# JackWoo0831/Yolov7-tracker

Measured on NVIDIA H100. Metric: tracked_frames_per_sec, higher is better.
Workload: dtype fp16

## Files before the change

### yolov7-tracker_b200/b200track/conv.py

```python
import ctypes as C

import torch

from . import _lib as L


def pack_conv_weight(w, cin_pad=None, dtype=torch.bfloat16):
    cout, cin, kh, kw = w.shape
    cin_pad = cin_pad or (cin + 15) // 16 * 16
    rows = (cout + 15) // 16 * 16
    out = torch.zeros((rows, kh, kw, cin_pad), dtype=torch.float32, device=w.device)
    out[:cout, :, :, :cin] = w.permute(0, 2, 3, 1)
    return out.reshape(rows, kh * kw * cin_pad).to(dtype).contiguous()


def pack_conv_weight_rowpack(w, dtype=torch.bfloat16):
    cout, cin, kh, kw = w.shape
    assert kh == 3 and kw == 3 and cin <= 16
    rows = (cout + 15) // 16 * 16
    out = torch.zeros((rows, 3, 4, 16), dtype=torch.float32, device=w.device)
    out[:cout, :, :3, :cin] = w.permute(0, 2, 3, 1)
    return out.reshape(rows, 192).to(dtype).contiguous()


class ConvPlan:
    def __init__(self, x, w_packed, bias, y, n, h, w, cin, in_coff, cout, k, stride, out_coff, act=True, out_f32=False,
                 block_n=0, tile_w=0, stages=0, in_row_pixels=0, rowpack=False, x_pixel0=0, halo=False, mt=1, splits=1, halo_bufs=0, producers=0, tps=0, out_bufs=0, kpair=0):
        self.lib = L.load()
        assert x.dtype in (torch.bfloat16, torch.float16) and x.is_contiguous() and y.is_contiguous()
        assert w_packed.dtype == x.dtype and bias.dtype == torch.float32 and (out_f32 or y.dtype == x.dtype)
        self.keep = (x, w_packed, bias, y)
        self.geom = dict(n=n, h=h, w=w, cin=cin, cout=cout, k=k, stride=stride, out_f32=bool(out_f32), rowpack=bool(rowpack))
        d = L.ConvDesc(x=x.data_ptr() + x_pixel0 * x.shape[-1] * 2, w_packed=w_packed.data_ptr(), bias=bias.data_ptr(), y=y.data_ptr(), n=n, h=h, w=w,
                       cin=cin, in_pitch=x.shape[-1], in_coff=in_coff, cout=cout, cout_rows=w_packed.shape[0], kh=k, kw=k,
                       stride=stride, out_pitch=y.shape[-1], out_coff=out_coff, act=int(act), out_f32=int(out_f32),
                       block_n=block_n, tile_w=tile_w, stages=stages, in_row_pixels=in_row_pixels, rowpack=int(rowpack), io_dtype=L.act_dtype_code(x.dtype),
                       halo=int(halo), halo_bufs=int(halo_bufs), tps=int(tps), kpair=int(kpair), out_bufs=int(out_bufs), mt=int(mt), producers=int(producers), splits=int(splits))
        self.handle = C.c_void_p()
        rc = self.lib.b2t_conv_plan_create(C.byref(d), C.byref(self.handle))
        if rc != 0:
            raise L.B2TError("b2t_conv_plan_create: %s" % (self.lib.b2t_conv_last_error() or b"").decode())
        self.flops = self.lib.b2t_conv_plan_flops(self.handle)
        info = (C.c_int * 17)()
        self.lib.b2t_conv_plan_info(self.handle, info, 17)
        self.info = dict(zip(("grid", "threads", "smem", "bn", "stages", "mt", "splits", "halo", "halo_bufs", "tiles_m", "tiles_n", "acc_regs", "producers", "tps", "b_res", "out_bufs", "kpair"), list(info)))

    def run(self, stream=None):
        s = C.c_void_p(torch.cuda.current_stream().cuda_stream if stream is None else stream)
        rc = self.lib.b2t_conv_run(self.handle, s)
        if rc != 0:
            raise L.B2TError("b2t_conv_run: %s" % (self.lib.b2t_conv_last_error() or b"").decode())

    def __del__(self):
        try:
            if self.handle:
                self.lib.b2t_conv_plan_destroy(self.handle)
                self.handle = None
        except Exception:
            pass
```

### yolov7-tracker_b200/csrc/b2t_conv.cu

```cuda
#include <cuda.h>
#include <cuda_runtime.h>
#include <cuda_bf16.h>
#include <cuda_fp16.h>
#include <stdint.h>
#include <string>
#include <cstdio>
#include <cstdlib>
#include "../../include/b200track.h"
#include "b2t_wgmma.cuh"

namespace {

constexpr int kMaxStages = 8;
constexpr int kTileM = 128;
constexpr int kMaxHalo = 3;
constexpr int kRing = 4;
constexpr int kMaxProducers = 2;

struct ConvParams {
    int N, H, W, Cin;
    int Ho, Wo, Cout;
    int KH, KW, stride, pad;
    int pad_w;
    int halo;
    int halo_bytes;
    int halo_bufs;
    int kpair;
    int tps;
    int b_res;
    int out_bufs;
    int MT;
    int sub_off;
    int TH, TW;
    int BK;
    int BN;
    int tiles_w, tiles_h;
    int out_pitch;
    int out_coff;
    int act;
    float act_floor, act_slope;
    int out_f32;
    int f16;
    int flat;
    int stages;
    int tiles_m, tiles_n;
    int P;
    int splits;
    int ksteps;
    long long total_pix;
    float* ws;
    int* flags;
};

__device__ __forceinline__ uint32_t smem_u32(const void* p) { return (uint32_t)__cvta_generic_to_shared(p); }

__device__ __forceinline__ void mbar_init(uint64_t* bar, int count) {
    asm volatile("mbarrier.init.shared::cta.b64 [%0], %1;" ::"r"(smem_u32(bar)), "r"(count));
}
__device__ __forceinline__ void mbar_expect_tx(uint64_t* bar, uint32_t bytes) {
    asm volatile("mbarrier.arrive.expect_tx.shared::cta.b64 _, [%0], %1;" ::"r"(smem_u32(bar)), "r"(bytes) : "memory");
}
__device__ __forceinline__ void mbar_arrive(uint64_t* bar) {
    asm volatile("mbarrier.arrive.shared::cta.b64 _, [%0];" ::"r"(smem_u32(bar)) : "memory");
}
__device__ __forceinline__ void mbar_wait(uint64_t* bar, uint32_t parity) {
    asm volatile(
        "{\n\t.reg .pred p;\n\t"
        "WAIT_%=:\n\t"
        "mbarrier.try_wait.parity.shared::cta.b64 p, [%0], %1;\n\t"
        "@p bra DONE_%=;\n\t"
        "bra WAIT_%=;\n\t"
        "DONE_%=:\n\t}" ::"r"(smem_u32(bar)), "r"(parity) : "memory");
}
__device__ __forceinline__ void tma_load_4d(void* dst, const CUtensorMap* map, uint64_t* bar, int c0, int c1, int c2, int c3) {
    asm volatile(
        "cp.async.bulk.tensor.4d.shared::cluster.global.tile.mbarrier::complete_tx::bytes [%0], [%1, {%3, %4, %5, %6}], [%2];"
        ::"r"(smem_u32(dst)), "l"(map), "r"(smem_u32(bar)), "r"(c0), "r"(c1), "r"(c2), "r"(c3) : "memory");
}
__device__ __forceinline__ void tma_load_2d(void* dst, const CUtensorMap* map, uint64_t* bar, int c0, int c1) {
    asm volatile(
        "cp.async.bulk.tensor.2d.shared::cluster.global.tile.mbarrier::complete_tx::bytes [%0], [%1, {%3, %4}], [%2];"
        ::"r"(smem_u32(dst)), "l"(map), "r"(smem_u32(bar)), "r"(c0), "r"(c1) : "memory");
}
__device__ __forceinline__ void tma_load_3d(void* dst, const CUtensorMap* map, uint64_t* bar, int c0, int c1, int c2) {
    asm volatile(
        "cp.async.bulk.tensor.3d.shared::cluster.global.tile.mbarrier::complete_tx::bytes [%0], [%1, {%3, %4, %5}], [%2];"
        ::"r"(smem_u32(dst)), "l"(map), "r"(smem_u32(bar)), "r"(c0), "r"(c1), "r"(c2) : "memory");
}
__device__ __forceinline__ void tma_store_4d(const CUtensorMap* map, const void* src, int c0, int c1, int c2, int c3) {
    asm volatile("cp.async.bulk.tensor.4d.global.shared::cta.bulk_group [%0, {%2, %3, %4, %5}], [%1];"
                 ::"l"(map), "r"(smem_u32(src)), "r"(c0), "r"(c1), "r"(c2), "r"(c3) : "memory");
}
__device__ __forceinline__ void tma_store_2d(const CUtensorMap* map, const void* src, int c0, int c1) {
    asm volatile("cp.async.bulk.tensor.2d.global.shared::cta.bulk_group [%0, {%2, %3}], [%1];"
                 ::"l"(map), "r"(smem_u32(src)), "r"(c0), "r"(c1) : "memory");
}
__device__ __forceinline__ bool elect_one() {
    uint32_t pred;
    asm volatile("{\n\t.reg .pred p;\n\telect.sync _|p, 0xffffffff;\n\tselp.u32 %0, 1, 0, p;\n\t}" : "=r"(pred));
    return pred != 0;
}
__device__ __forceinline__ void wgmma_fence() { asm volatile("wgmma.fence.sync.aligned;" ::: "memory"); }
__device__ __forceinline__ void wgmma_commit() { asm volatile("wgmma.commit_group.sync.aligned;" ::: "memory"); }
template <int N> __device__ __forceinline__ void wgmma_wait() { asm volatile("wgmma.wait_group.sync.aligned %0;" ::"n"(N) : "memory"); }
template <int R> __device__ __forceinline__ void acc_fence(float (&d)[R]) {
#pragma unroll
    for (int i = 0; i < R; ++i) asm volatile("" : "+f"(d[i])::"memory");
}

__device__ __forceinline__ float silu(float v) {
    const float h = 0.5f * v;
    float t;
    asm("tanh.approx.f32 %0, %1;" : "=f"(t) : "f"(h));
    return fmaf(h, t, h);
}

__device__ __forceinline__ uint32_t pack16(float a, float b, bool f16) {
    if (f16) { const __half2 h = __floats2half2_rn(a, b); return *reinterpret_cast<const uint32_t*>(&h); }
    const __nv_bfloat162 h = __floats2bfloat162_rn(a, b); return *reinterpret_cast<const uint32_t*>(&h);
}

template <bool F32, bool F16, int BN>
__device__ __forceinline__ void stage_box(const float (&acc)[BN / 2], int bx, const float* __restrict__ bias_c, uint8_t* box, int r0, int lane,
                                          int act, float floor_v, float slope_v) {
    constexpr int cpb = F32 ? 32 : 64;
    const int cq = 2 * (lane & 3);
#pragma unroll
    for (int j = 0; j < BN / 8; ++j) {
        if ((8 * j) / cpb != bx) continue;
        const int col = 8 * j + cq;
        const float2 b = __ldg(reinterpret_cast<const float2*>(bias_c + col));
#pragma unroll
        for (int h = 0; h < 2; ++h) {
            const int r = r0 + 8 * h;
            float v0 = acc[4 * j + 2 * h] + b.x, v1 = acc[4 * j + 2 * h + 1] + b.y;
            if (act) { v0 = silu(v0); v1 = silu(v1); }
            else {
                v0 = fmaxf(fmaxf(v0, floor_v), v0 * slope_v); v1 = fmaxf(fmaxf(v1, floor_v), v1 * slope_v);
            }
            const int byte = (col - bx * cpb) * (F32 ? 4 : 2);
            uint8_t* dst = box + r * 128 + ((((byte >> 4) ^ (r & 7)) << 4) | (byte & 15));
            if (F32) *reinterpret_cast<float2*>(dst) = make_float2(v0, v1);
            else *reinterpret_cast<uint32_t*>(dst) = pack16(v0, v1, F16);
        }
    }
}

template <bool F32, bool F16, int MT, int BN>
__global__ void __launch_bounds__(256 * MT + 32 * kMaxProducers, (MT == 1 && BN <= 64) ? 2 : 1)
conv_bias_act_kernel(const __grid_constant__ CUtensorMap map_a, const __grid_constant__ CUtensorMap map_b,
                     const __grid_constant__ CUtensorMap map_c, const float* __restrict__ bias, int* __restrict__ sched,
                     const ConvParams p) {
    extern __shared__ __align__(1024) uint8_t smem[];
    constexpr int kConsumerWarps = 8 * MT;
    const int warp = threadIdx.x >> 5, lane = threadIdx.x & 31;
    const int a_bytes = kTileM * p.BK * 2;
    const int b_bytes = BN * p.BK * 2;
    const int stage_bytes = (((p.halo ? p.tps * b_bytes : (MT * a_bytes + b_bytes) * p.kpair) + 1023) / 1024) * 1024;
    uint8_t* tiles = smem + ((1024u - (smem_u32(smem) & 1023u)) & 1023u);
    uint8_t* ring = tiles + (p.halo ? p.halo_bufs * p.halo_bytes : 0);
    const int kStages = p.stages;
    constexpr int box_bytes = kTileM * 128;
    const int staging_bytes = p.out_bufs * box_bytes;
    uint8_t* stage_out = ring + kStages * stage_bytes;
    uint64_t* full_bar = reinterpret_cast<uint64_t*>(stage_out + MT * staging_bytes);
    uint64_t* empty_bar = full_bar + kMaxStages;
    uint64_t* ring_full = empty_bar + kMaxStages;
    uint64_t* ring_empty = ring_full + kRing;
    uint64_t* a_full = ring_empty + kRing;
    uint64_t* a_empty = a_full + kMaxHalo;
    int* tile_ring = reinterpret_cast<int*>(a_empty + kMaxHalo);
    int* last_flag = tile_ring + kRing;
    int* first_unit = last_flag + 2;

    const int ntaps = p.KH * p.KW;
    const int total_units = p.tiles_m * p.tiles_n * p.splits;
    const int P = p.P;
    const int pw = warp - kConsumerWarps;

    asm volatile("griddepcontrol.launch_dependents;" ::: "memory");
    if (pw == 0 && lane == 0) {
        *first_unit = atomicAdd(sched, 1);
        asm volatile("prefetch.tensormap [%0];" ::"l"(&map_a) : "memory");
        asm volatile("prefetch.tensormap [%0];" ::"l"(&map_b) : "memory");
        asm volatile("prefetch.tensormap [%0];" ::"l"(&map_c) : "memory");
        for (int s = 0; s < kStages; ++s) { mbar_init(&full_bar[s], 1); mbar_init(&empty_bar[s], 2 * MT); }
        for (int r = 0; r < kRing; ++r) { mbar_init(&ring_full[r], 1); mbar_init(&ring_empty[r], P - 1 + kConsumerWarps); }
        for (int h = 0; h < kMaxHalo; ++h) { mbar_init(&a_full[h], 1); mbar_init(&a_empty[h], 2 * MT); }
        asm volatile("fence.mbarrier_init.release.cluster;" ::: "memory");
    }
    __syncthreads();

    auto unit_coords = [&](int u, int& n0, int& img, int& ho0, int& wo0, long long& pix0, int& k0, int& k1) {
        int t = u;
        k0 = 0; k1 = p.ksteps;
        if (p.splits > 1) {
            t = u / p.splits;
            const int sp = u - t * p.splits;
            k0 = (p.ksteps * sp) / p.splits;
            k1 = (p.ksteps * (sp + 1)) / p.splits;
        }
        const int mt = t / p.tiles_n, nt = t % p.tiles_n;
        n0 = nt * BN; img = 0; ho0 = 0; wo0 = 0; pix0 = 0;
        if (p.flat) pix0 = (long long)mt * (kTileM * MT);
        else {
            const int per_img = p.tiles_w * p.tiles_h;
            img = mt / per_img;
            const int r = mt % per_img;
            ho0 = (r / p.tiles_w) * (p.halo ? p.TH : p.TH * MT);
            wo0 = (r % p.tiles_w) * (p.halo ? p.TW * MT : p.TW);
        }
    };

    if (pw >= 0) {
        int stage = 0; uint32_t phase = 0;
        int hbuf = 0; uint32_t hphase = 0;
        int rslot = 0; uint32_t rphase = 0;
        int c = 0;
        int u = *first_unit;
        const int groups = p.halo ? 9 / p.tps : 1;
        auto load_b = [&](int st, int n0, int k0, int s) {
            uint8_t* sb = ring + st * stage_bytes + (p.halo ? 0 : MT * a_bytes * p.kpair);
            if (p.halo) {
                const int kc = k0 + s / groups, tap = (s % groups) * p.tps;
                if (p.tps == 1) tma_load_2d(sb, &map_b, &full_bar[st], tap * p.Cin + kc * p.BK, n0);
                else tma_load_3d(sb, &map_b, &full_bar[st], kc * p.BK, n0, tap);
            } else if (p.kpair == 2) {
                tma_load_3d(sb, &map_b, &full_bar[st], 0, n0, 2 * (k0 + s));
            } else {
                const int kt = k0 + s, kc = kt / ntaps, tap = kt % ntaps;
                tma_load_2d(sb, &map_b, &full_bar[st], tap * p.Cin + kc * p.BK, n0);
            }
        };
        const uint32_t stage_tx = (uint32_t)(p.halo ? p.tps * b_bytes : (MT * a_bytes + b_bytes) * p.kpair);
        int npre = 0;
        if (u < total_units) {
            int n0, img, ho0, wo0, k0, k1; long long pix0;
            unit_coords(u, n0, img, ho0, wo0, pix0, k0, k1);
            if (p.b_res) {
                if (pw == 0 && elect_one()) {
                    mbar_expect_tx(&full_bar[0], (uint32_t)(9 * b_bytes));
                    tma_load_3d(ring, &map_b, &full_bar[0], 0, n0, 0);
                }
            } else {
                const int nsteps = (k1 - k0) * groups;
                npre = nsteps < kStages ? nsteps : kStages;
                for (int s = pw; s < npre; s += P)
                    if (elect_one()) {
                        mbar_expect_tx(&full_bar[s], stage_tx);
                        load_b(s, n0, k0, s);
                    }
            }
            __syncwarp();
        }
        asm volatile("griddepcontrol.wait;" ::: "memory");
        for (;;) {
            if (pw == 0) {
                const bool live = u < total_units;
                mbar_wait(&ring_empty[rslot], rphase ^ 1);
                if (lane == 0) {
                    tile_ring[rslot] = live ? u : -1;
                    mbar_arrive(&ring_full[rslot]);
                }
                __syncwarp();
                if (++rslot == kRing) { rslot = 0; rphase ^= 1; }
                if (!live) break;
            } else {
                mbar_wait(&ring_full[rslot], rphase);
                u = tile_ring[rslot];
                __syncwarp();
                if (lane == 0) mbar_arrive(&ring_empty[rslot]);
                if (++rslot == kRing) { rslot = 0; rphase ^= 1; }
                if (u < 0) break;
            }
            int next = 0;
            if (pw == 0) {
                if (lane == 0) next = atomicAdd(sched, 1);
                next = __shfl_sync(0xffffffffu, next, 0);
            }
            int n0, img, ho0, wo0, k0, k1; long long pix0;
            unit_coords(u, n0, img, ho0, wo0, pix0, k0, k1);
            if (p.halo) {
                const uint32_t halo_tx = (uint32_t)((p.TW * MT + 2) * (p.TH + 2) * p.BK * 2);
                auto load_halo = [&](int kc) {
                    mbar_wait(&a_empty[hbuf], hphase ^ 1);
                    if (elect_one()) {
                        mbar_expect_tx(&a_full[hbuf], halo_tx);
                        tma_load_4d(tiles + hbuf * p.halo_bytes, &map_a, &a_full[hbuf], kc * p.BK, wo0 - 1, ho0 - 1, img);
                    }
                    __syncwarp();
                    if (++hbuf == p.halo_bufs) { hbuf = 0; hphase ^= 1; }
                };
                if (pw == 0) load_halo(k0);
                for (int kc = k0; kc < k1; ++kc) {
                    if (pw == 0 && kc + 1 < k1) load_halo(kc + 1);
                    if (p.b_res) continue;
                    for (int g = 0; g < groups; ++g, ++c) {
                        if (c % P == pw && c >= npre) {
                            mbar_wait(&empty_bar[stage], phase ^ 1);
                            if (elect_one()) {
                                mbar_expect_tx(&full_bar[stage], stage_tx);
                                load_b(stage, n0, kc, g);
                            }
                            __syncwarp();
                        }
                        if (++stage == kStages) { stage = 0; phase ^= 1; }
                    }
                }
            } else
            for (int kt = k0; kt < k1; ++kt, ++c) {
                if (c % P == pw) {
                    const int kc = kt / ntaps, tap = kt % ntaps;
                    const int kh = tap / p.KW, kw = tap % p.KW;
                    const bool pre = c < npre;
                    mbar_wait(&empty_bar[stage], phase ^ 1);
                    if (elect_one()) {
                        uint8_t* sa = ring + stage * stage_bytes;
                        if (!pre) mbar_expect_tx(&full_bar[stage], stage_tx);
                        if (p.kpair == 2) tma_load_3d(sa, &map_a, &full_bar[stage], 0, (int)pix0, 2 * kt);
                        else if (p.flat) tma_load_2d(sa, &map_a, &full_bar[stage], kc * p.BK, (int)pix0);
                        else tma_load_4d(sa, &map_a, &full_bar[stage], kc * p.BK, wo0 * p.stride + kw - p.pad_w, ho0 * p.stride + kh - p.pad, img);
                        if (!pre) load_b(stage, n0, kt, 0);
                    }
                    __syncwarp();
                }
                if (++stage == kStages) { stage = 0; phase ^= 1; }
            }
            u = next;
        }
        if (pw == 0 && lane == 0 && atomicAdd(sched + 1, 1) == (int)gridDim.x - 1) {
            sched[0] = 0; sched[1] = 0;
            __threadfence();
        }
    } else {
        const int g = warp >> 3;
        const int hh = (warp >> 2) & 1;
        const int gtid = (int)threadIdx.x - g * 256;
        const int bar_id = 1 + g;
        const bool wg_leader = (threadIdx.x & 127) == 0;
        const int r0 = hh * 64 + (warp & 3) * 16 + (lane >> 2);
        const int row_bytes = p.BK * 2;
        const int halo_w = p.TW * MT + 2;
        const uint32_t layout = row_bytes == 128 ? 1u : (row_bytes == 64 ? 2u : 3u);
        const uint32_t hi_b = (uint32_t)((8 * row_bytes) >> 4) | (layout << 30);
        const uint32_t hi_a = p.halo ? ((uint32_t)((halo_w * row_bytes) >> 4) | (layout << 30)) : hi_b;
        const uint32_t ring_lo = ((smem_u32(ring) >> 4) & 0x3fffu) | (1u << 16);
        const uint32_t tiles_lo = ((smem_u32(tiles) >> 4) & 0x3fffu) | (1u << 16);
        const uint32_t stage_step = (uint32_t)stage_bytes >> 4, halo_step = (uint32_t)p.halo_bytes >> 4;
        const uint32_t b_off = (uint32_t)(MT * a_bytes) >> 4, b_step = (uint32_t)b_bytes >> 4;
        const uint32_t row_step = (uint32_t)row_bytes >> 4;
        const uint32_t a_off = (uint32_t)(g * p.sub_off) / 16u + (uint32_t)hh * (p.halo ? 8u * (uint32_t)halo_w * row_step : 64u * row_step);
        auto desc = [](uint32_t lo, uint32_t hi) { return ((uint64_t)hi << 32) | lo; };
        const int ksub = p.BK / 16;
        bool b_ready = false;
        int stage = 0; uint32_t phase = 0;
        int hbuf = 0; uint32_t hphase = 0;
        int rslot = 0; uint32_t rphase = 0;
        constexpr int cols_per_box = F32 ? 32 : 64;
        constexpr int nboxes = (BN + cols_per_box - 1) / cols_per_box;
        int box_seq = 0;
        float acc[BN / 2];
        for (;;) {
            mbar_wait(&ring_full[rslot], rphase);
            const int u = tile_ring[rslot];
            __syncwarp();
            if (lane == 0) mbar_arrive(&ring_empty[rslot]);
            if (++rslot == kRing) { rslot = 0; rphase ^= 1; }
            if (u < 0) break;
            int n0, img, ho0, wo0, k0, k1; long long pix0;
            unit_coords(u, n0, img, ho0, wo0, pix0, k0, k1);
            int pend_stage = -1, pend_halo = -1;
            auto release = [&](int st, int hb) {
                if (wg_leader) {
                    if (st >= 0) mbar_arrive(&empty_bar[st]);
                    if (hb >= 0) mbar_arrive(&a_empty[hb]);
                }
            };
            auto retire = [&](int st, int hb, bool drain) {
                if (drain) {
                    wgmma_wait<0>();
                    acc_fence(acc);
                    release(pend_stage, pend_halo);
                    release(st, hb);
                    pend_stage = pend_halo = -1;
                } else {
                    wgmma_wait<1>();
                    acc_fence(acc);
                    release(pend_stage, pend_halo);
                    pend_stage = st; pend_halo = hb;
                }
            };
            uint32_t scale = 0;
            if (p.halo) {
                for (int kc = k0; kc < k1; ++kc) {
                    mbar_wait(&a_full[hbuf], hphase);
                    const uint32_t a_buf = tiles_lo + (uint32_t)hbuf * halo_step + a_off;
                    for (int tap0 = 0; tap0 < 9; tap0 += p.tps) {
                        if (!p.b_res || !b_ready) {
                            mbar_wait(&full_bar[stage], phase);
                            b_ready = true;
                        }
                        const uint32_t b_stage = ring_lo + (uint32_t)stage * stage_step;
                        acc_fence(acc);
                        wgmma_fence();
                        for (int t = 0; t < p.tps; ++t) {
                            const int tap = tap0 + t, kh = tap / 3, kw = tap - 3 * kh;
                            const uint32_t a_lo = a_buf + (uint32_t)(kh * halo_w + kw) * row_step;
                            const uint32_t b_lo = b_stage + (uint32_t)t * b_step;
                            for (int k = 0; k < ksub; ++k) {
                                wgmma_m64k16<BN, F16>(acc, desc(a_lo + 2u * k, hi_a), desc(b_lo + 2u * k, hi_b), scale);
                                scale = 1;
                            }
                        }
                        wgmma_commit();
                        const bool chunk_end = tap0 + p.tps >= 9;
                        retire(p.b_res ? -1 : stage, chunk_end ? hbuf : -1, chunk_end || kStages == 1);
                        if (!p.b_res && ++stage == kStages) { stage = 0; phase ^= 1; }
                    }
                    if (++hbuf == p.halo_bufs) { hbuf = 0; hphase ^= 1; }
                }
            } else
            for (int kt = k0; kt < k1; ++kt) {
                mbar_wait(&full_bar[stage], phase);
                const uint32_t a_st = ring_lo + (uint32_t)stage * stage_step;
                const uint32_t b_st = a_st + b_off * (uint32_t)p.kpair;
                acc_fence(acc);
                wgmma_fence();
                for (int j = 0; j < p.kpair; ++j) {
                    const uint32_t a_lo = a_st + (uint32_t)j * b_off + a_off, b_lo = b_st + (uint32_t)j * b_step;
                    for (int k = 0; k < ksub; ++k) {
                        wgmma_m64k16<BN, F16>(acc, desc(a_lo + 2u * k, hi_a), desc(b_lo + 2u * k, hi_b), scale);
                        scale = 1;
                    }
                }
                wgmma_commit();
                retire(stage, -1, kStages == 1);
                if (++stage == kStages) { stage = 0; phase ^= 1; }
            }
            wgmma_wait<0>();
            acc_fence(acc);
            release(pend_stage, pend_halo);
            const long long gpix = pix0 + (long long)g * kTileM;
            const int gho = p.halo ? ho0 : ho0 + g * p.TH;
            const int gwo = p.halo ? wo0 + g * p.TW : wo0;
            const bool in_range = p.flat ? (gpix < p.total_pix) : (gho < p.Ho && gwo < p.Wo);
            bool reduce_here = true;
            if (p.splits > 1) {
                const int cq = 2 * (lane & 3);
                float* wsub = p.ws + ((size_t)u * MT + g) * kTileM * BN;
#pragma unroll
                for (int j = 0; j < BN / 8; ++j)
#pragma unroll
                    for (int h = 0; h < 2; ++h)
                        __stcg(reinterpret_cast<float2*>(wsub + (size_t)(r0 + 8 * h) * BN + 8 * j + cq), make_float2(acc[4 * j + 2 * h], acc[4 * j + 2 * h + 1]));
                __threadfence();
                asm volatile("bar.sync %0, 256;" ::"r"(bar_id) : "memory");
                if (gtid == 0) {
                    const int t = u / p.splits;
                    const int old = atomicAdd(p.flags + t * MT + g, 1);
                    const int last = old == p.splits - 1;
                    if (last) p.flags[t * MT + g] = 0;
                    last_flag[g] = last;
                }
                asm volatile("bar.sync %0, 256;" ::"r"(bar_id) : "memory");
                reduce_here = last_flag[g] != 0;
                if (reduce_here) {
                    __threadfence();
                    const int t = u / p.splits;
#pragma unroll
                    for (int i = 0; i < BN / 2; ++i) acc[i] = 0.f;
                    for (int sp = 0; sp < p.splits; ++sp) {
                        const float* src = p.ws + (((size_t)t * p.splits + sp) * MT + g) * kTileM * BN;
#pragma unroll
                        for (int j = 0; j < BN / 8; ++j)
#pragma unroll
                            for (int h = 0; h < 2; ++h) {
                                const float2 x = __ldcg(reinterpret_cast<const float2*>(src + (size_t)(r0 + 8 * h) * BN + 8 * j + cq));
                                acc[4 * j + 2 * h] += x.x; acc[4 * j + 2 * h + 1] += x.y;
                            }
                    }
                }
            }
            if (reduce_here) {
                const float* bias_t = bias + n0;
#pragma unroll
                for (int bx = 0; bx < nboxes; ++bx, ++box_seq) {
                    uint8_t* stage_cur = stage_out + g * staging_bytes + (p.out_bufs == 2 ? (box_seq & 1) * box_bytes : 0);
                    if (gtid == 0) {
                        if (p.out_bufs == 2) asm volatile("cp.async.bulk.wait_group.read 1;" ::: "memory");
                        else asm volatile("cp.async.bulk.wait_group.read 0;" ::: "memory");
                    }
                    asm volatile("bar.sync %0, 256;" ::"r"(bar_id) : "memory");
                    if (in_range) stage_box<F32, F16, BN>(acc, bx, bias_t, stage_cur, r0, lane, p.act, p.act_floor, p.act_slope);
                    asm volatile("fence.proxy.async.shared::cta;" ::: "memory");
                    asm volatile("bar.sync %0, 256;" ::"r"(bar_id) : "memory");
                    if (gtid == 0) {
                        const int cc = n0 + bx * cols_per_box;
                        if (in_range && cc < p.Cout) {
                            if (p.flat) tma_store_2d(&map_c, stage_cur, cc, (int)gpix);
                            else tma_store_4d(&map_c, stage_cur, cc, gwo, gho, img);
                        }
                        asm volatile("cp.async.bulk.commit_group;" ::: "memory");
                    }
                }
            }
        }
        if (gtid == 0) asm volatile("cp.async.bulk.wait_group.read 0;" ::: "memory");
    }
}

thread_local std::string g_conv_err;
int cfail(int code, const std::string& m) { g_conv_err = m; return code; }

typedef CUresult (*EncodeTiledFn)(CUtensorMap*, CUtensorMapDataType, cuuint32_t, void*, const cuuint64_t*, const cuuint64_t*,
                                  const cuuint32_t*, const cuuint32_t*, CUtensorMapInterleave, CUtensorMapSwizzle,
                                  CUtensorMapL2promotion, CUtensorMapFloatOOBfill);
EncodeTiledFn get_encode() {
    static EncodeTiledFn fn = nullptr;
    if (!fn) {
        void* p = nullptr;
        cudaDriverEntryPointQueryResult q;
        if (cudaGetDriverEntryPoint("cuTensorMapEncodeTiled", &p, cudaEnableDefault, &q) == cudaSuccess && q == cudaDriverEntryPointSuccess)
            fn = reinterpret_cast<EncodeTiledFn>(p);
    }
    return fn;
}
CUtensorMapSwizzle swizzle_for(int bk) {
    return bk == 64 ? CU_TENSOR_MAP_SWIZZLE_128B : (bk == 32 ? CU_TENSOR_MAP_SWIZZLE_64B : CU_TENSOR_MAP_SWIZZLE_32B);
}

}

typedef void (*ConvKernelFn)(const CUtensorMap, const CUtensorMap, const CUtensorMap, const float*, int*, const ConvParams);

struct b2t_conv_plan {
    ConvKernelFn kernel;
    CUtensorMap map_a, map_b, map_c;
    ConvParams p;
    float* bias_pad;
    double flops;
    int* sched;
    mutable unsigned launches;
    float* ws;
    int* flags;
    void* out;
    dim3 grid;
    int threads;
    size_t smem;
};

template <bool F32, bool F16>
ConvKernelFn kernel_for_bn(int mt, int bn) {
    if (mt == 1) {
        switch (bn) {
            case 32: return conv_bias_act_kernel<F32, F16, 1, 32>;
            case 64: return conv_bias_act_kernel<F32, F16, 1, 64>;
            case 128: return conv_bias_act_kernel<F32, F16, 1, 128>;
            case 256: return conv_bias_act_kernel<F32, F16, 1, 256>;
        }
    } else if (mt == 2) {
        switch (bn) {
            case 32: return conv_bias_act_kernel<F32, F16, 2, 32>;
            case 64: return conv_bias_act_kernel<F32, F16, 2, 64>;
            case 128: return conv_bias_act_kernel<F32, F16, 2, 128>;
        }
    }
    return nullptr;
}
ConvKernelFn kernel_for(int f32, int f16, int mt, int bn) {
    if (f16) return f32 ? kernel_for_bn<true, true>(mt, bn) : kernel_for_bn<false, true>(mt, bn);
    return f32 ? kernel_for_bn<true, false>(mt, bn) : kernel_for_bn<false, false>(mt, bn);
}

extern "C" const char* b2t_conv_last_error(void) { return g_conv_err.c_str(); }

static void free_plan(b2t_conv_plan* pl) {
    if (!pl) return;
    if (pl->bias_pad) cudaFree(pl->bias_pad);
// ... 84 lines not shown
                CU_TENSOR_MAP_L2_PROMOTION_L2_128B, CU_TENSOR_MAP_FLOAT_OOB_FILL_NONE);
    } else if (p.flat) {
        cuuint64_t dims[2] = {(cuuint64_t)p.Cin, (cuuint64_t)p.total_pix};
        cuuint64_t strides[1] = {(cuuint64_t)d->in_pitch * 2};
        cuuint32_t box[2] = {(cuuint32_t)bk, (cuuint32_t)(kTileM * MT)};
        cuuint32_t es[2] = {1, 1};
        r = enc(&pl->map_a, dt16, 2, a_base, dims, strides, box, es, CU_TENSOR_MAP_INTERLEAVE_NONE, sw,
                CU_TENSOR_MAP_L2_PROMOTION_L2_128B, CU_TENSOR_MAP_FLOAT_OOB_FILL_NONE);
    } else {
        cuuint64_t dims[4] = {(cuuint64_t)p.Cin, (cuuint64_t)p.W, (cuuint64_t)p.H, (cuuint64_t)p.N};
        cuuint64_t strides[3] = {(cuuint64_t)d->in_pitch * 2, (cuuint64_t)d->in_pitch * 2 * row_pixels, (cuuint64_t)d->in_pitch * 2 * row_pixels * p.H};
        cuuint32_t box[4] = {(cuuint32_t)bk, (cuuint32_t)(p.TW * p.stride), (cuuint32_t)(p.TH * MT * p.stride), 1};
        if (halo) { box[1] = (cuuint32_t)(p.TW * MT + 2); box[2] = (cuuint32_t)(p.TH + 2); }
        cuuint32_t es[4] = {1, (cuuint32_t)p.stride, (cuuint32_t)p.stride, 1};
        r = enc(&pl->map_a, dt16, 4, a_base, dims, strides, box, es, CU_TENSOR_MAP_INTERLEAVE_NONE, sw,
                CU_TENSOR_MAP_L2_PROMOTION_L2_128B, CU_TENSOR_MAP_FLOAT_OOB_FILL_NONE);
    }
    if (r != CUDA_SUCCESS) { free_plan(pl); return cfail(B2T_ECUDA, "cuTensorMapEncodeTiled(A) failed: " + std::to_string((int)r)); }
    const int kchunks_h = p.Cin / bk;
    const int tiles_n_pre = (cout_pad + bn - 1) / bn;
    int tps = 1;
    p.b_res = 0;
    if (halo) {
        tps = d->tps > 0 ? d->tps : (bn <= 128 ? 3 : 1);
        if (tps != 1 && tps != 3 && tps != 9) { free_plan(pl); return cfail(B2T_EINVAL, "b2t_conv_plan_create: tps must be 1, 3 or 9"); }
        if ((d->tps == 0 || d->tps == 9) && kchunks_h == 1 && tiles_n_pre == 1 && splits == 1 && 9 * bn * bk * 2 <= 96 * 1024) { tps = 9; p.b_res = 1; }
        else if (tps == 9) { free_plan(pl); return cfail(B2T_EINVAL, "b2t_conv_plan_create: tps = 9 (resident weights) needs one K chunk, one N tile and <= 96 KB of weights"); }
    }
    p.tps = tps;
    {
        const cuuint64_t K = (cuuint64_t)p.KH * p.KW * p.Cin;
        if (p.kpair == 2) {
            cuuint64_t dims[3] = {64, (cuuint64_t)d->cout_rows, (cuuint64_t)(p.Cin / 64)};
            cuuint64_t strides[2] = {K * 2, 128};
            cuuint32_t box[3] = {64, (cuuint32_t)bn, 2};
            cuuint32_t es[3] = {1, 1, 1};
            r = enc(&pl->map_b, dt16, 3, const_cast<void*>(d->w_packed), dims, strides, box, es,
                    CU_TENSOR_MAP_INTERLEAVE_NONE, sw, CU_TENSOR_MAP_L2_PROMOTION_L2_256B, CU_TENSOR_MAP_FLOAT_OOB_FILL_NONE);
        } else if (tps > 1) {
            cuuint64_t dims[3] = {(cuuint64_t)p.Cin, (cuuint64_t)d->cout_rows, 9};
            cuuint64_t strides[2] = {K * 2, (cuuint64_t)p.Cin * 2};
            cuuint32_t box[3] = {(cuuint32_t)bk, (cuuint32_t)bn, (cuuint32_t)tps};
            cuuint32_t es[3] = {1, 1, 1};
            r = enc(&pl->map_b, dt16, 3, const_cast<void*>(d->w_packed), dims, strides, box, es,
                    CU_TENSOR_MAP_INTERLEAVE_NONE, sw, CU_TENSOR_MAP_L2_PROMOTION_L2_256B, CU_TENSOR_MAP_FLOAT_OOB_FILL_NONE);
        } else {
            cuuint64_t dims[2] = {K, (cuuint64_t)d->cout_rows};
            cuuint64_t strides[1] = {K * 2};
            cuuint32_t box[2] = {(cuuint32_t)bk, (cuuint32_t)bn};
            cuuint32_t es[2] = {1, 1};
            r = enc(&pl->map_b, dt16, 2, const_cast<void*>(d->w_packed), dims, strides, box, es,
                    CU_TENSOR_MAP_INTERLEAVE_NONE, sw, CU_TENSOR_MAP_L2_PROMOTION_L2_256B, CU_TENSOR_MAP_FLOAT_OOB_FILL_NONE);
        }
        if (r != CUDA_SUCCESS) { free_plan(pl); return cfail(B2T_ECUDA, "cuTensorMapEncodeTiled(B) failed: " + std::to_string((int)r)); }
    }
    {
        const int esize = p.out_f32 ? 4 : 2;
        const CUtensorMapDataType dt = p.out_f32 ? CU_TENSOR_MAP_DATA_TYPE_FLOAT32 : dt16;
        char* c_base = reinterpret_cast<char*>(d->y) + (size_t)d->out_coff * esize;
        const cuuint32_t cb = 128 / esize;
        if (((uintptr_t)c_base & 15) || ((size_t)d->out_pitch * esize) % 16) { free_plan(pl); return cfail(B2T_EINVAL, "b2t_conv_plan_create: output slice must be 16-byte aligned"); }
        if (p.flat) {
            cuuint64_t dims[2] = {(cuuint64_t)p.Cout, (cuuint64_t)p.total_pix};
            cuuint64_t strides[1] = {(cuuint64_t)d->out_pitch * esize};
            cuuint32_t box[2] = {cb, (cuuint32_t)kTileM};
            cuuint32_t es[2] = {1, 1};
            r = enc(&pl->map_c, dt, 2, c_base, dims, strides, box, es, CU_TENSOR_MAP_INTERLEAVE_NONE, CU_TENSOR_MAP_SWIZZLE_128B,
                    CU_TENSOR_MAP_L2_PROMOTION_NONE, CU_TENSOR_MAP_FLOAT_OOB_FILL_NONE);
        } else {
            cuuint64_t dims[4] = {(cuuint64_t)p.Cout, (cuuint64_t)p.Wo, (cuuint64_t)p.Ho, (cuuint64_t)p.N};
            cuuint64_t strides[3] = {(cuuint64_t)d->out_pitch * esize, (cuuint64_t)d->out_pitch * esize * p.Wo, (cuuint64_t)d->out_pitch * esize * p.Wo * p.Ho};
            cuuint32_t box[4] = {cb, (cuuint32_t)p.TW, (cuuint32_t)p.TH, 1};
            cuuint32_t es[4] = {1, 1, 1, 1};
            r = enc(&pl->map_c, dt, 4, c_base, dims, strides, box, es, CU_TENSOR_MAP_INTERLEAVE_NONE, CU_TENSOR_MAP_SWIZZLE_128B,
                    CU_TENSOR_MAP_L2_PROMOTION_NONE, CU_TENSOR_MAP_FLOAT_OOB_FILL_NONE);
        }
        if (r != CUDA_SUCCESS) { free_plan(pl); return cfail(B2T_ECUDA, "cuTensorMapEncodeTiled(C) failed: " + std::to_string((int)r)); }
    }
    const int a_bytes = kTileM * bk * 2, b_bytes = bn * bk * 2;
    const int stage_bytes = (((halo ? tps * b_bytes : (MT * a_bytes + b_bytes) * p.kpair) + 1023) / 1024) * 1024;
    if (halo) { p.halo_bytes = ((p.TW * MT + 2) * (p.TH + 2) * bk * 2 + 1023) / 1024 * 1024; p.halo_bufs = 2; }
    const int box_bytes = kTileM * 128;
    p.out_bufs = d->out_bufs == 1 ? 1 : 2;
    auto smem_for = [&](int st) { return (size_t)p.halo_bufs * p.halo_bytes + (size_t)st * stage_bytes + (size_t)MT * p.out_bufs * box_bytes + 512 + 1024; };
    ConvKernelFn kfn = kernel_for(p.out_f32, p.f16, MT, bn);
    if (!kfn) { free_plan(pl); return cfail(B2T_EINVAL, "b2t_conv_plan_create: no kernel for this mt / BLOCK_N"); }
    if (cudaFuncSetAttribute(kfn, cudaFuncAttributeMaxDynamicSharedMemorySize, 227 * 1024) != cudaSuccess) {
        free_plan(pl); return cfail(B2T_ECUDA, "cannot raise dynamic shared memory for conv kernel");
    }
    cudaFuncAttributes fa;
    if (cudaFuncGetAttributes(&fa, kfn) != cudaSuccess) { free_plan(pl); return cfail(B2T_ECUDA, "cudaFuncGetAttributes(conv kernel) failed"); }
    const bool two_by_regs = 2 * fa.numRegs * (256 * MT + 32 * kMaxProducers) <= 65536;
    int stages = d->stages > 0 ? (d->stages < kMaxStages ? d->stages : kMaxStages) : 0;
    if (p.b_res) stages = 1;
    const int min_stages = (halo || p.kpair == 2) ? 2 : 3;
    if (stages == 0) {
        for (int pass = 0; pass < 2 && stages == 0; ++pass) {
            int per2 = 0, per1 = 0;
            for (int st = kMaxStages; st >= 1; --st) { if (!per2 && smem_for(st) <= 113 * 1024) per2 = st; if (!per1 && smem_for(st) <= 226 * 1024) per1 = st; }
            const int pick = (two_by_regs && MT == 1 && per2 >= 3) ? per2 : per1;
            if (pick >= min_stages || p.out_bufs == 1 || d->out_bufs == 2) stages = pick;
            else p.out_bufs = 1;
        }
        if (stages < 1) stages = 1;
    }
    while (stages > 1 && smem_for(stages) > 226 * 1024) --stages;
    if (smem_for(stages) > 226 * 1024 && p.out_bufs == 2) p.out_bufs = 1;
    if (smem_for(stages) > 227 * 1024) { free_plan(pl); return cfail(B2T_EINVAL, "b2t_conv_plan_create: tile does not fit in shared memory (reduce BLOCK_N, mt or tps)"); }
    if (halo && d->halo_bufs == 3 && smem_for(stages) + p.halo_bytes <= 226 * 1024) p.halo_bufs = 3;
    const int P_eff = P > stages ? stages : P;
    p.P = P_eff;
    const int threads = 256 * MT + 32 * P_eff;
    p.stages = stages;
    pl->smem = smem_for(stages);
    pl->threads = threads;
    int ctas_per_sm = 1;
    if (cudaOccupancyMaxActiveBlocksPerMultiprocessor(&ctas_per_sm, kfn, threads, pl->smem) != cudaSuccess || ctas_per_sm < 1) ctas_per_sm = 1;
    p.tiles_m = p.flat ? (int)((p.total_pix + kTileM * MT - 1) / (kTileM * MT)) : p.N * p.tiles_w * p.tiles_h;
    p.tiles_n = (cout_pad + bn - 1) / bn;
    int n_sm = 132;
    { int devid = 0; cudaGetDevice(&devid); int v = 0; if (cudaDeviceGetAttribute(&v, cudaDevAttrMultiProcessorCount, devid) == cudaSuccess && v > 0) n_sm = v; }
    const long long total_units = (long long)p.tiles_m * p.tiles_n * splits;
    if (total_units > 0x7fffffff) { free_plan(pl); return cfail(B2T_EINVAL, "b2t_conv_plan_create: too many tiles"); }
    long long g = (long long)n_sm * ctas_per_sm;
    if (g > total_units) g = total_units;
    pl->grid = dim3((unsigned)g, 1, 1);
    pl->kernel = kfn;
    {
        const size_t nb = (size_t)p.tiles_n * bn + 64;
        if (cudaMalloc(&pl->bias_pad, nb * sizeof(float)) != cudaSuccess) { free_plan(pl); return cfail(B2T_ECUDA, "cudaMalloc(bias) failed"); }
        if (cudaMemset(pl->bias_pad, 0, nb * sizeof(float)) != cudaSuccess ||
            cudaMemcpy(pl->bias_pad, d->bias, (size_t)d->cout * sizeof(float), cudaMemcpyDeviceToDevice) != cudaSuccess) {
            free_plan(pl); return cfail(B2T_ECUDA, "bias snapshot failed");
        }
        if (cudaMalloc(&pl->sched, 8 * sizeof(int)) != cudaSuccess || cudaMemset(pl->sched, 0, 8 * sizeof(int)) != cudaSuccess) {
            free_plan(pl); return cfail(B2T_ECUDA, "cudaMalloc(tile counters) failed");
        }
    }
    if (splits > 1) {
        const size_t wsb = (size_t)total_units * MT * kTileM * bn * sizeof(float);
        const size_t nf = (size_t)p.tiles_m * p.tiles_n * MT * sizeof(int);
        if (cudaMalloc(&pl->ws, wsb) != cudaSuccess || cudaMalloc(&pl->flags, nf) != cudaSuccess || cudaMemset(pl->flags, 0, nf) != cudaSuccess) {
            free_plan(pl); return cfail(B2T_ECUDA, "cudaMalloc(split-K workspace) failed");
        }
    }
    p.ws = pl->ws; p.flags = pl->flags;
    *out_plan = pl;
    return B2T_OK;
}

extern "C" void b2t_conv_plan_destroy(b2t_conv_plan* pl) { free_plan(pl); }

extern "C" double b2t_conv_plan_flops(const b2t_conv_plan* pl) { return pl ? pl->flops : 0.0; }

extern "C" int b2t_conv_plan_info(const b2t_conv_plan* pl, int* out, int n) {
    if (!pl || !out) return cfail(B2T_EINVAL, "b2t_conv_plan_info: null argument");
    const ConvParams& p = pl->p;
    const int v[17] = {(int)pl->grid.x, pl->threads, (int)pl->smem, p.BN, p.stages, p.MT, p.splits, p.halo, p.halo_bufs, p.tiles_m, p.tiles_n, p.BN / 2, p.P,
                       p.tps, p.b_res, p.out_bufs, p.kpair};
    for (int i = 0; i < n && i < 17; ++i) out[i] = v[i];
    return B2T_OK;
}

extern "C" int b2t_conv_run(const b2t_conv_plan* pl, void* stream) {
    if (!pl) return cfail(B2T_EINVAL, "b2t_conv_run: null plan");
    static const bool use_pdl = [] { const char* v = getenv("B2T_CONV_PDL"); return !(v && v[0] == '0'); }();
    cudaLaunchConfig_t cfg = {};
    cfg.gridDim = pl->grid; cfg.blockDim = dim3(pl->threads); cfg.dynamicSmemBytes = pl->smem; cfg.stream = (cudaStream_t)stream;
    cudaLaunchAttribute attr[1];
    attr[0].id = cudaLaunchAttributeProgrammaticStreamSerialization;
    attr[0].val.programmaticStreamSerializationAllowed = 1;
    cfg.attrs = attr; cfg.numAttrs = use_pdl ? 1 : 0;
    cudaError_t e = cudaLaunchKernelEx(&cfg, pl->kernel, pl->map_a, pl->map_b, pl->map_c, (const float*)pl->bias_pad,
                                       pl->sched + 2 * (pl->launches++ & 3u), pl->p);
    if (e == cudaSuccess) e = cudaGetLastError();
    if (e != cudaSuccess) return cfail(B2T_ECUDA, std::string("conv launch: ") + cudaGetErrorString(e));
    return B2T_OK;
}
```

Baseline: 761.6.

## Add ping-pong consumer warpgroups with setmaxnreg register hand-off in conv kernel

For MT==1 and BN<=128 each consumer warpgroup now owns a whole 128-row tile (two m64 halves) and the two warpgroups alternate tiles, taking turns on the MMA via mbarriers. This lets one group's epilogue overlap with the other's MMA mainloop. Producer warps shrink their registers with setmaxnreg and consumers grow theirs, with a fixed producer warpgroup size. Occupancy is forced to 1 CTA/SM and smem staging doubles, which may cost small layers that previously ran 2 CTAs per SM.

Result: faster. 811.1 (median of 6 runs) (+6.5%).

```diff
diff --git a/yolov7-tracker_b200/b200track/conv.py b/yolov7-tracker_b200/b200track/conv.py
--- a/yolov7-tracker_b200/b200track/conv.py
+++ b/yolov7-tracker_b200/b200track/conv.py
@@ -41,9 +41,9 @@
         if rc != 0:
             raise L.B2TError("b2t_conv_plan_create: %s" % (self.lib.b2t_conv_last_error() or b"").decode())
         self.flops = self.lib.b2t_conv_plan_flops(self.handle)
-        info = (C.c_int * 17)()
-        self.lib.b2t_conv_plan_info(self.handle, info, 17)
-        self.info = dict(zip(("grid", "threads", "smem", "bn", "stages", "mt", "splits", "halo", "halo_bufs", "tiles_m", "tiles_n", "acc_regs", "producers", "tps", "b_res", "out_bufs", "kpair"), list(info)))
+        info = (C.c_int * 18)()
+        self.lib.b2t_conv_plan_info(self.handle, info, 18)
+        self.info = dict(zip(("grid", "threads", "smem", "bn", "stages", "mt", "splits", "halo", "halo_bufs", "tiles_m", "tiles_n", "acc_regs", "producers", "tps", "b_res", "out_bufs", "kpair", "pingpong"), list(info)))
 
     def run(self, stream=None):
         s = C.c_void_p(torch.cuda.current_stream().cuda_stream if stream is None else stream)
diff --git a/yolov7-tracker_b200/csrc/b2t_conv.cu b/yolov7-tracker_b200/csrc/b2t_conv.cu
--- a/yolov7-tracker_b200/csrc/b2t_conv.cu
+++ b/yolov7-tracker_b200/csrc/b2t_conv.cu
@@ -16,6 +16,13 @@
 constexpr int kMaxHalo = 3;
 constexpr int kRing = 4;
 constexpr int kMaxProducers = 2;
+
+__host__ __device__ constexpr bool ping_pong(int mt, int bn) { return mt == 1 && bn <= 128; }
+__host__ __device__ constexpr int conv_threads(int mt) { return 256 * mt + 128; }
+__host__ __device__ constexpr int launch_regs(int mt) { return 65536 / conv_threads(mt) / 8 * 8; }
+constexpr int kProducerRegs = 48;
+__host__ __device__ constexpr int consumer_regs(int mt) { return (launch_regs(mt) + (launch_regs(mt) - kProducerRegs) * 128 / (256 * mt)) / 8 * 8; }
+static_assert(consumer_regs(1) == 224 && consumer_regs(2) == 104, "register hand-off");
 
 struct ConvParams {
     int N, H, W, Cin;
@@ -103,10 +110,15 @@
 __device__ __forceinline__ void wgmma_fence() { asm volatile("wgmma.fence.sync.aligned;" ::: "memory"); }
 __device__ __forceinline__ void wgmma_commit() { asm volatile("wgmma.commit_group.sync.aligned;" ::: "memory"); }
 template <int N> __device__ __forceinline__ void wgmma_wait() { asm volatile("wgmma.wait_group.sync.aligned %0;" ::"n"(N) : "memory"); }
-template <int R> __device__ __forceinline__ void acc_fence(float (&d)[R]) {
-#pragma unroll
-    for (int i = 0; i < R; ++i) asm volatile("" : "+f"(d[i])::"memory");
-}
+template <int H, int R> __device__ __forceinline__ void acc_fence(float (&d)[H][R]) {
+#pragma unroll
+    for (int h = 0; h < H; ++h)
+#pragma unroll
+        for (int i = 0; i < R; ++i) asm volatile("" : "+f"(d[h][i])::"memory");
+}
+template <int N> struct Steps { static constexpr int value = N; };
+template <int N> __device__ __forceinline__ void setmaxnreg_dec() { asm volatile("setmaxnreg.dec.sync.aligned.u32 %0;" ::"n"(N)); }
+template <int N> __device__ __forceinline__ void setmaxnreg_inc() { asm volatile("setmaxnreg.inc.sync.aligned.u32 %0;" ::"n"(N)); }
 
 __device__ __forceinline__ float silu(float v) {
     const float h = 0.5f * v;
@@ -147,12 +159,14 @@
 }
 
 template <bool F32, bool F16, int MT, int BN>
-__global__ void __launch_bounds__(256 * MT + 32 * kMaxProducers, (MT == 1 && BN <= 64) ? 2 : 1)
+__global__ void __launch_bounds__(conv_threads(MT), 1)
 conv_bias_act_kernel(const __grid_constant__ CUtensorMap map_a, const __grid_constant__ CUtensorMap map_b,
                      const __grid_constant__ CUtensorMap map_c, const float* __restrict__ bias, int* __restrict__ sched,
                      const ConvParams p) {
     extern __shared__ __align__(1024) uint8_t smem[];
     constexpr int kConsumerWarps = 8 * MT;
+    constexpr bool kPingPong = ping_pong(MT, BN);
+    constexpr int kSlots = kPingPong ? 2 : MT;
     const int warp = threadIdx.x >> 5, lane = threadIdx.x & 31;
     const int a_bytes = kTileM * p.BK * 2;
     const int b_bytes = BN * p.BK * 2;
@@ -163,13 +177,14 @@
     constexpr int box_bytes = kTileM * 128;
     const int staging_bytes = p.out_bufs * box_bytes;
     uint8_t* stage_out = ring + kStages * stage_bytes;
-    uint64_t* full_bar = reinterpret_cast<uint64_t*>(stage_out + MT * staging_bytes);
+    uint64_t* full_bar = reinterpret_cast<uint64_t*>(stage_out + kSlots * staging_bytes);
     uint64_t* empty_bar = full_bar + kMaxStages;
     uint64_t* ring_full = empty_bar + kMaxStages;
     uint64_t* ring_empty = ring_full + kRing;
     uint64_t* a_full = ring_empty + kRing;
     uint64_t* a_empty = a_full + kMaxHalo;
-    int* tile_ring = reinterpret_cast<int*>(a_empty + kMaxHalo);
+    uint64_t* mma_turn = a_empty + kMaxHalo;
+    int* tile_ring = reinterpret_cast<int*>(mma_turn + 2);
     int* last_flag = tile_ring + kRing;
     int* first_unit = last_flag + 2;
 
@@ -184,9 +199,11 @@
         asm volatile("prefetch.tensormap [%0];" ::"l"(&map_a) : "memory");
         asm volatile("prefetch.tensormap [%0];" ::"l"(&map_b) : "memory");
         asm volatile("prefetch.tensormap [%0];" ::"l"(&map_c) : "memory");
-        for (int s = 0; s < kStages; ++s) { mbar_init(&full_bar[s], 1); mbar_init(&empty_bar[s], 2 * MT); }
+        constexpr int readers = kPingPong ? 1 : 2 * MT;
+        for (int s = 0; s < kStages; ++s) { mbar_init(&full_bar[s], 1); mbar_init(&empty_bar[s], readers); }
         for (int r = 0; r < kRing; ++r) { mbar_init(&ring_full[r], 1); mbar_init(&ring_empty[r], P - 1 + kConsumerWarps); }
-        for (int h = 0; h < kMaxHalo; ++h) { mbar_init(&a_full[h], 1); mbar_init(&a_empty[h], 2 * MT); }
+        for (int h = 0; h < kMaxHalo; ++h) { mbar_init(&a_full[h], 1); mbar_init(&a_empty[h], readers); }
+        for (int w = 0; w < 2; ++w) mbar_init(&mma_turn[w], 1);
         asm volatile("fence.mbarrier_init.release.cluster;" ::: "memory");
     }
     __syncthreads();
@@ -213,6 +230,8 @@
     };
 
     if (pw >= 0) {
+        setmaxnreg_dec<kProducerRegs>();
+        if (pw >= P) return;
         int stage = 0; uint32_t phase = 0;
         int hbuf = 0; uint32_t hphase = 0;
         int rslot = 0; uint32_t rphase = 0;
@@ -333,12 +352,17 @@
             __threadfence();
         }
     } else {
-        const int g = warp >> 3;
-        const int hh = (warp >> 2) & 1;
-        const int gtid = (int)threadIdx.x - g * 256;
-        const int bar_id = 1 + g;
+        setmaxnreg_inc<consumer_regs(MT)>();
+        constexpr int kHalves = kPingPong ? 2 : 1;
+        constexpr int kGroupThreads = kPingPong ? 128 : 256;
+        const int wg = warp >> 2;
+        const int slot = kPingPong ? wg : warp >> 3;
+        const int g = kPingPong ? 0 : warp >> 3;
+        const int hh0 = kPingPong ? 0 : wg & 1;
+        const int gtid = (int)threadIdx.x - slot * kGroupThreads;
+        const int bar_id = 1 + slot;
         const bool wg_leader = (threadIdx.x & 127) == 0;
-        const int r0 = hh * 64 + (warp & 3) * 16 + (lane >> 2);
+        const int rw = (warp & 3) * 16 + (lane >> 2);
         const int row_bytes = p.BK * 2;
         const int halo_w = p.TW * MT + 2;
         const uint32_t layout = row_bytes == 128 ? 1u : (row_bytes == 64 ? 2u : 3u);
@@ -349,7 +373,8 @@
         const uint32_t stage_step = (uint32_t)stage_bytes >> 4, halo_step = (uint32_t)p.halo_bytes >> 4;
         const uint32_t b_off = (uint32_t)(MT * a_bytes) >> 4, b_step = (uint32_t)b_bytes >> 4;
         const uint32_t row_step = (uint32_t)row_bytes >> 4;
-        const uint32_t a_off = (uint32_t)(g * p.sub_off) / 16u + (uint32_t)hh * (p.halo ? 8u * (uint32_t)halo_w * row_step : 64u * row_step);
+        const uint32_t half_step = p.halo ? 8u * (uint32_t)halo_w * row_step : 64u * row_step;
+        const uint32_t a_off = (uint32_t)(g * p.sub_off) / 16u + (uint32_t)hh0 * half_step;
         auto desc = [](uint32_t lo, uint32_t hi) { return ((uint64_t)hi << 32) | lo; };
         const int ksub = p.BK / 16;
         bool b_ready = false;
@@ -359,7 +384,10 @@
         constexpr int cols_per_box = F32 ? 32 : 64;
         constexpr int nboxes = (BN + cols_per_box - 1) / cols_per_box;
         int box_seq = 0;
-        float acc[BN / 2];
+        int entry = 0;
+        int turns = 0;
+        auto advance = [](int& pos, uint32_t& ph, int n, int len) { const int t = pos + n; ph ^= (uint32_t)((t / len) & 1); pos = t % len; };
+        float acc[kHalves][BN / 2];
         for (;;) {
             mbar_wait(&ring_full[rslot], rphase);
             const int u = tile_ring[rslot];
@@ -369,6 +397,16 @@
             if (u < 0) break;
             int n0, img, ho0, wo0, k0, k1; long long pix0;
             unit_coords(u, n0, img, ho0, wo0, pix0, k0, k1);
+            if (kPingPong && (entry++ & 1) != wg) {
+                if (p.halo) {
+                    advance(hbuf, hphase, k1 - k0, p.halo_bufs);
+                    if (!p.b_res) advance(stage, phase, (k1 - k0) * (9 / p.tps), kStages);
+                } else {
+                    advance(stage, phase, k1 - k0, kStages);
+                }
+                continue;
+            }
+            if (kPingPong && (wg == 1 || turns > 0)) mbar_wait(&mma_turn[wg], (uint32_t)((wg == 0 ? turns - 1 : turns) & 1));
             int pend_stage = -1, pend_halo = -1;
             auto release = [&](int st, int hb) {
                 if (wg_leader) {
@@ -391,6 +429,20 @@
                 }
             };
             uint32_t scale = 0;
+            auto chain = [&](auto ksteps, uint32_t a_lo, uint32_t b_lo) {
+#pragma unroll
+                for (int k = 0; k < decltype(ksteps)::value; ++k) {
+#pragma unroll
+                    for (int h = 0; h < kHalves; ++h)
+                        wgmma_m64k16<BN, F16>(acc[h], desc(a_lo + (uint32_t)h * half_step + 2u * k, hi_a), desc(b_lo + 2u * k, hi_b), scale);
+                    scale = 1;
+                }
+            };
+            auto mma_chunk = [&](uint32_t a_lo, uint32_t b_lo) {
+                if (ksub == 4) chain(Steps<4>{}, a_lo, b_lo);
+                else if (ksub == 2) chain(Steps<2>{}, a_lo, b_lo);
+                else chain(Steps<1>{}, a_lo, b_lo);
+            };
             if (p.halo) {
                 for (int kc = k0; kc < k1; ++kc) {
                     mbar_wait(&a_full[hbuf], hphase);
@@ -407,10 +459,7 @@
                             const int tap = tap0 + t, kh = tap / 3, kw = tap - 3 * kh;
                             const uint32_t a_lo = a_buf + (uint32_t)(kh * halo_w + kw) * row_step;
                             const uint32_t b_lo = b_stage + (uint32_t)t * b_step;
-                            for (int k = 0; k < ksub; ++k) {
-                                wgmma_m64k16<BN, F16>(acc, desc(a_lo + 2u * k, hi_a), desc(b_lo + 2u * k, hi_b), scale);
-                                scale = 1;
-                            }
+                            mma_chunk(a_lo, b_lo);
                         }
                         wgmma_commit();
                         const bool chunk_end = tap0 + p.tps >= 9;
@@ -428,14 +477,15 @@
                 wgmma_fence();
                 for (int j = 0; j < p.kpair; ++j) {
                     const uint32_t a_lo = a_st + (uint32_t)j * b_off + a_off, b_lo = b_st + (uint32_t)j * b_step;
-                    for (int k = 0; k < ksub; ++k) {
-                        wgmma_m64k16<BN, F16>(acc, desc(a_lo + 2u * k, hi_a), desc(b_lo + 2u * k, hi_b), scale);
-                        scale = 1;
-                    }
+                    mma_chunk(a_lo, b_lo);
                 }
                 wgmma_commit();
                 retire(stage, -1, kStages == 1);
                 if (++stage == kStages) { stage = 0; phase ^= 1; }
+            }
+            if (kPingPong) {
+                if (wg_leader) mbar_arrive(&mma_turn[wg ^ 1]);
+                ++turns;
             }
             wgmma_wait<0>();
             acc_fence(acc);
@@ -449,35 +499,45 @@
                 const int cq = 2 * (lane & 3);
                 float* wsub = p.ws + ((size_t)u * MT + g) * kTileM * BN;
 #pragma unroll
-                for (int j = 0; j < BN / 8; ++j)
-#pragma unroll
-                    for (int h = 0; h < 2; ++h)
-                        __stcg(reinterpret_cast<float2*>(wsub + (size_t)(r0 + 8 * h) * BN + 8 * j + cq), make_float2(acc[4 * j + 2 * h], acc[4 * j + 2 * h + 1]));
+                for (int hf = 0; hf < kHalves; ++hf) {
+                    const int r0 = (hh0 + hf) * 64 + rw;
+#pragma unroll
+                    for (int j = 0; j < BN / 8; ++j)
+#pragma unroll
+                        for (int h = 0; h < 2; ++h)
+                            __stcg(reinterpret_cast<float2*>(wsub + (size_t)(r0 + 8 * h) * BN + 8 * j + cq), make_float2(acc[hf][4 * j + 2 * h], acc[hf][4 * j + 2 * h + 1]));
+                }
                 __threadfence();
-                asm volatile("bar.sync %0, 256;" ::"r"(bar_id) : "memory");
+                asm volatile("bar.sync %0, %1;" ::"r"(bar_id), "n"(kGroupThreads) : "memory");
                 if (gtid == 0) {
                     const int t = u / p.splits;
                     const int old = atomicAdd(p.flags + t * MT + g, 1);
                     const int last = old == p.splits - 1;
                     if (last) p.flags[t * MT + g] = 0;
-                    last_flag[g] = last;
-                }
-                asm volatile("bar.sync %0, 256;" ::"r"(bar_id) : "memory");
-                reduce_here = last_flag[g] != 0;
+                    last_flag[slot] = last;
+                }
+                asm volatile("bar.sync %0, %1;" ::"r"(bar_id), "n"(kGroupThreads) : "memory");
+                reduce_here = last_flag[slot] != 0;
                 if (reduce_here) {
                     __threadfence();
                     const int t = u / p.splits;
 #pragma unroll
-                    for (int i = 0; i < BN / 2; ++i) acc[i] = 0.f;
+                    for (int hf = 0; hf < kHalves; ++hf)
+#pragma unroll
+                        for (int i = 0; i < BN / 2; ++i) acc[hf][i] = 0.f;
                     for (int sp = 0; sp < p.splits; ++sp) {
                         const float* src = p.ws + (((size_t)t * p.splits + sp) * MT + g) * kTileM * BN;
 #pragma unroll
-                        for (int j = 0; j < BN / 8; ++j)
-#pragma unroll
-                            for (int h = 0; h < 2; ++h) {
-                                const float2 x = __ldcg(reinterpret_cast<const float2*>(src + (size_t)(r0 + 8 * h) * BN + 8 * j + cq));
-                                acc[4 * j + 2 * h] += x.x; acc[4 * j + 2 * h + 1] += x.y;
-                            }
+                        for (int hf = 0; hf < kHalves; ++hf) {
+                            const int r0 = (hh0 + hf) * 64 + rw;
+#pragma unroll
+                            for (int j = 0; j < BN / 8; ++j)
+#pragma unroll
+                                for (int h = 0; h < 2; ++h) {
+                                    const float2 x = __ldcg(reinterpret_cast<const float2*>(src + (size_t)(r0 + 8 * h) * BN + 8 * j + cq));
+                                    acc[hf][4 * j + 2 * h] += x.x; acc[hf][4 * j + 2 * h + 1] += x.y;
+                                }
+                        }
                     }
                 }
             }
@@ -485,15 +545,19 @@
                 const float* bias_t = bias + n0;
 #pragma unroll
                 for (int bx = 0; bx < nboxes; ++bx, ++box_seq) {
-                    uint8_t* stage_cur = stage_out + g * staging_bytes + (p.out_bufs == 2 ? (box_seq & 1) * box_bytes : 0);
+                    uint8_t* stage_cur = stage_out + slot * staging_bytes + (p.out_bufs == 2 ? (box_seq & 1) * box_bytes : 0);
                     if (gtid == 0) {
                         if (p.out_bufs == 2) asm volatile("cp.async.bulk.wait_group.read 1;" ::: "memory");
                         else asm volatile("cp.async.bulk.wait_group.read 0;" ::: "memory");
                     }
-                    asm volatile("bar.sync %0, 256;" ::"r"(bar_id) : "memory");
-                    if (in_range) stage_box<F32, F16, BN>(acc, bx, bias_t, stage_cur, r0, lane, p.act, p.act_floor, p.act_slope);
+                    asm volatile("bar.sync %0, %1;" ::"r"(bar_id), "n"(kGroupThreads) : "memory");
+                    if (in_range) {
+#pragma unroll
+                        for (int hf = 0; hf < kHalves; ++hf)
+                            stage_box<F32, F16, BN>(acc[hf], bx, bias_t, stage_cur, (hh0 + hf) * 64 + rw, lane, p.act, p.act_floor, p.act_slope);
+                    }
                     asm volatile("fence.proxy.async.shared::cta;" ::: "memory");
-                    asm volatile("bar.sync %0, 256;" ::"r"(bar_id) : "memory");
+                    asm volatile("bar.sync %0, %1;" ::"r"(bar_id), "n"(kGroupThreads) : "memory");
                     if (gtid == 0) {
                         const int cc = n0 + bx * cols_per_box;
                         if (in_range && cc < p.Cout) {
@@ -744,23 +808,21 @@
     if (halo) { p.halo_bytes = ((p.TW * MT + 2) * (p.TH + 2) * bk * 2 + 1023) / 1024 * 1024; p.halo_bufs = 2; }
     const int box_bytes = kTileM * 128;
     p.out_bufs = d->out_bufs == 1 ? 1 : 2;
-    auto smem_for = [&](int st) { return (size_t)p.halo_bufs * p.halo_bytes + (size_t)st * stage_bytes + (size_t)MT * p.out_bufs * box_bytes + 512 + 1024; };
+    const int slots = ping_pong(MT, bn) ? 2 : MT;
+    auto smem_for = [&](int st) { return (size_t)p.halo_bufs * p.halo_bytes + (size_t)st * stage_bytes + (size_t)slots * p.out_bufs * box_bytes + 512 + 1024; };
     ConvKernelFn kfn = kernel_for(p.out_f32, p.f16, MT, bn);
     if (!kfn) { free_plan(pl); return cfail(B2T_EINVAL, "b2t_conv_plan_create: no kernel for this mt / BLOCK_N"); }
     if (cudaFuncSetAttribute(kfn, cudaFuncAttributeMaxDynamicSharedMemorySize, 227 * 1024) != cudaSuccess) {
         free_plan(pl); return cfail(B2T_ECUDA, "cannot raise dynamic shared memory for conv kernel");
     }
-    cudaFuncAttributes fa;
-    if (cudaFuncGetAttributes(&fa, kfn) != cudaSuccess) { free_plan(pl); return cfail(B2T_ECUDA, "cudaFuncGetAttributes(conv kernel) failed"); }
-    const bool two_by_regs = 2 * fa.numRegs * (256 * MT + 32 * kMaxProducers) <= 65536;
+    const int threads = conv_threads(MT);
     int stages = d->stages > 0 ? (d->stages < kMaxStages ? d->stages : kMaxStages) : 0;
     if (p.b_res) stages = 1;
     const int min_stages = (halo || p.kpair == 2) ? 2 : 3;
     if (stages == 0) {
         for (int pass = 0; pass < 2 && stages == 0; ++pass) {
-            int per2 = 0, per1 = 0;
-            for (int st = kMaxStages; st >= 1; --st) { if (!per2 && smem_for(st) <= 113 * 1024) per2 = st; if (!per1 && smem_for(st) <= 226 * 1024) per1 = st; }
-            const int pick = (two_by_regs && MT == 1 && per2 >= 3) ? per2 : per1;
+            int pick = 0;
+            for (int st = kMaxStages; st >= 1 && !pick; --st) if (smem_for(st) <= 226 * 1024) pick = st;
             if (pick >= min_stages || p.out_bufs == 1 || d->out_bufs == 2) stages = pick;
             else p.out_bufs = 1;
         }
@@ -772,7 +834,6 @@
     if (halo && d->halo_bufs == 3 && smem_for(stages) + p.halo_bytes <= 226 * 1024) p.halo_bufs = 3;
     const int P_eff = P > stages ? stages : P;
     p.P = P_eff;
-    const int threads = 256 * MT + 32 * P_eff;
     p.stages = stages;
     pl->smem = smem_for(stages);
     pl->threads = threads;
@@ -818,9 +879,9 @@
 extern "C" int b2t_conv_plan_info(const b2t_conv_plan* pl, int* out, int n) {
     if (!pl || !out) return cfail(B2T_EINVAL, "b2t_conv_plan_info: null argument");
     const ConvParams& p = pl->p;
-    const int v[17] = {(int)pl->grid.x, pl->threads, (int)pl->smem, p.BN, p.stages, p.MT, p.splits, p.halo, p.halo_bufs, p.tiles_m, p.tiles_n, p.BN / 2, p.P,
-                       p.tps, p.b_res, p.out_bufs, p.kpair};
-    for (int i = 0; i < n && i < 17; ++i) out[i] = v[i];
+    const int v[18] = {(int)pl->grid.x, pl->threads, (int)pl->smem, p.BN, p.stages, p.MT, p.splits, p.halo, p.halo_bufs, p.tiles_m, p.tiles_n,
+                       p.BN / 2 * (ping_pong(p.MT, p.BN) ? 2 : 1), p.P, p.tps, p.b_res, p.out_bufs, p.kpair, ping_pong(p.MT, p.BN) ? 1 : 0};
+    for (int i = 0; i < n && i < 18; ++i) out[i] = v[i];
     return B2T_OK;
 }
 
```
